# 10XGenomics/lariat

Measured on AMD Instinct MI355X. Metric: read-pairs/sec aligned to hg38 (per-barcode align loop: SMEM seeding + SW + RFA/MAPQ on device); synthetic hg38-scale reference, higher is better.
Workload: dtype u64/i32 (FM-index + integer DP), f64 (RFA scores)

## Files before the change

include/lariat_hip.h:

```cpp
#ifndef LARIAT_HIP_H
#define LARIAT_HIP_H

#include <stddef.h>
#include <stdint.h>

#ifdef __cplusplus
extern "C" {
#endif

#define LH_ABI_VERSION 6

#define LH_OK 0
#define LH_E_ARG 1
#define LH_E_IO 2
#define LH_E_HIP 3
#define LH_E_CAPACITY 4
#define LH_E_NODEVICE 5
#define LH_E_LIMIT 6

#define LH_MAX_READ_LEN 250

typedef struct lh_index lh_index;
typedef struct lh_context lh_context;

typedef struct lh_opts {
    int32_t abi_version;
    int32_t a, b, o_del, e_del, o_ins, e_ins;
    int32_t pen_unpaired, pen_clip5, pen_clip3;
    int32_t w, zdrop, T;
    int32_t min_seed_len, min_chain_weight, max_chain_extend;
    float split_factor;
    int32_t split_width, max_occ, max_chain_gap, max_ins;
    float mask_level, drop_ratio, XA_drop_ratio, mask_level_redun;
    float mapQ_coef_len;
    int32_t max_mem_intv, max_matesw;
    int32_t pes_low, pes_high;
    int32_t rescue_score_delta;
    int32_t rescue_max_hits;
    int32_t aln_score_delta;
    double improper_pair_penalty;
    double genome_length;
    int32_t run_inference;
    uint32_t flags;
} lh_opts;

#define LH_F_NO_SWEEP_FILTER 1u
#define LH_F_EXT_WAVE 16u
#define LH_F_EXT_SERIAL 32u
#define LH_F_P2_TASKS 128u
#define LH_F_RESCUE_FULL 256u
#define LH_F_CHAIN_WAVE 64u

typedef struct lh_index_opts {
    int32_t abi_version;
    int32_t sa_intv;
    int32_t sb_shift;
    int32_t no_kmer_table;
    int32_t no_unique_runs;
    int32_t no_sweep_filter;
    int32_t build_chunk_log2;
    int32_t ktree_levels;
} lh_index_opts;
void lh_index_opts_init(lh_index_opts* io);

typedef struct lh_context_opts {
    int32_t abi_version;
    int32_t smem_grid;
    int32_t aln_grid;
    int32_t rfa_grid;
    int32_t rfa_slab_kb;
    int32_t lanes;
    int32_t big_slots;
    int32_t rfa_tier_kb[2];
    int32_t rfa_tier_grid[2];
    int32_t seed_budget_kb;
} lh_context_opts;
void lh_context_opts_init(lh_context_opts* co);

typedef struct lh_batch {
    int32_t n_barcodes;
    int32_t n_pairs;
    const int32_t* bc_pair_off;
    const uint8_t* bc_do_rfa;
    const int64_t* seq_off;
    const uint8_t* seq;
    const uint64_t* name_seed;
    const int64_t* cen_start;
    const int64_t* cen_end;
} lh_batch;

typedef struct lh_result {
    int32_t abi_version;
    int32_t n_reads;
    int64_t n_cand;
    const int64_t* cand_off;
    const int32_t* rid;
    const int64_t* pos;
    const int64_t* aend;
    const int64_t* rb;
    const int64_t* re;
    const uint8_t* reversed;
    const int32_t* score;
    const int32_t* qb;
// ... 210 lines not shown
```

lariat_amd/capi.py:

```python
import ctypes as C
import os

import numpy as np

_HERE = os.path.dirname(os.path.abspath(__file__))
LIB_PATH = os.environ.get("LARIAT_HIP_LIB") or os.path.join(_HERE, "_build", "liblariat_hip.so")

LH_OK = 0
LH_ABI_VERSION = 6
LH_E_ARG, LH_E_IO, LH_E_HIP, LH_E_CAPACITY, LH_E_NODEVICE, LH_E_LIMIT = 1, 2, 3, 4, 5, 6
LH_REC_DEBUG_TAGS = 1
LH_F_NO_SWEEP_FILTER, LH_F_EXT_WAVE, LH_F_EXT_SERIAL, LH_F_CHAIN_WAVE, LH_F_P2_TASKS, LH_F_RESCUE_FULL = 1, 16, 32, 64, 128, 256
LH_MAX_READ_LEN = 250

c_i32p = C.POINTER(C.c_int32)
c_i64p = C.POINTER(C.c_int64)
c_u8p = C.POINTER(C.c_uint8)
c_u32p = C.POINTER(C.c_uint32)
c_u64p = C.POINTER(C.c_uint64)
c_f64p = C.POINTER(C.c_double)


class LhOpts(C.Structure):
    _fields_ = [
        ("abi_version", C.c_int32),
        ("a", C.c_int32), ("b", C.c_int32), ("o_del", C.c_int32), ("e_del", C.c_int32), ("o_ins", C.c_int32), ("e_ins", C.c_int32),
        ("pen_unpaired", C.c_int32), ("pen_clip5", C.c_int32), ("pen_clip3", C.c_int32),
        ("w", C.c_int32), ("zdrop", C.c_int32), ("T", C.c_int32),
        ("min_seed_len", C.c_int32), ("min_chain_weight", C.c_int32), ("max_chain_extend", C.c_int32),
        ("split_factor", C.c_float),
        ("split_width", C.c_int32), ("max_occ", C.c_int32), ("max_chain_gap", C.c_int32), ("max_ins", C.c_int32),
        ("mask_level", C.c_float), ("drop_ratio", C.c_float), ("XA_drop_ratio", C.c_float), ("mask_level_redun", C.c_float),
        ("mapQ_coef_len", C.c_float),
        ("max_mem_intv", C.c_int32), ("max_matesw", C.c_int32),
        ("pes_low", C.c_int32), ("pes_high", C.c_int32),
        ("rescue_score_delta", C.c_int32), ("rescue_max_hits", C.c_int32), ("aln_score_delta", C.c_int32),
        ("improper_pair_penalty", C.c_double), ("genome_length", C.c_double),
        ("run_inference", C.c_int32), ("flags", C.c_uint32),
    ]


class LhIndexOpts(C.Structure):
    _fields_ = [("abi_version", C.c_int32), ("sa_intv", C.c_int32), ("sb_shift", C.c_int32), ("no_kmer_table", C.c_int32), ("no_unique_runs", C.c_int32),
                ("no_sweep_filter", C.c_int32), ("build_chunk_log2", C.c_int32), ("ktree_levels", C.c_int32)]


class LhContextOpts(C.Structure):
    _fields_ = [("abi_version", C.c_int32), ("smem_grid", C.c_int32), ("aln_grid", C.c_int32), ("rfa_grid", C.c_int32), ("rfa_slab_kb", C.c_int32),
                ("lanes", C.c_int32), ("big_slots", C.c_int32), ("rfa_tier_kb", C.c_int32 * 2), ("rfa_tier_grid", C.c_int32 * 2), ("seed_budget_kb", C.c_int32)]


class LhRoundInfo(C.Structure):
    _fields_ = [("n_rounds", C.c_int32), ("max_barcode", C.c_int32), ("first_barcode", c_i32p), ("round_seeds", c_i64p), ("round_need_bytes", c_i64p),
                ("need_bytes", C.c_int64), ("budget_bytes", C.c_int64), ("max_barcode_need_bytes", C.c_int64)]


class LhBatch(C.Structure):
    _fields_ = [
        ("n_barcodes", C.c_int32), ("n_pairs", C.c_int32),
        ("bc_pair_off", c_i32p), ("bc_do_rfa", c_u8p),
        ("seq_off", c_i64p), ("seq", c_u8p), ("name_seed", c_u64p),
        ("cen_start", c_i64p), ("cen_end", c_i64p),
    ]


# ... 888 lines not shown
```

lariat_amd/csrc/k_seed.h:

```cpp
#pragma once
#include "lh_dev.h"

struct DSeed { i64 rbeg; int32_t qbeg, len; };

#define LH_SCAN_TILE 2048
__device__ __forceinline__ i64 scan_val(const int32_t* in, int i, int n, int add, int at_least) {
    if (i >= n) return 0;
    i64 v = (i64)in[i] + add;
    return v < at_least ? at_least : v;
}
__global__ void __launch_bounds__(256) k_scan_partial(int n, const int32_t* __restrict__ in, int add, int at_least, i64* __restrict__ tile_sum) {
    __shared__ i64 part[256];
    int t = threadIdx.x, base = blockIdx.x * LH_SCAN_TILE + t * 8;
    i64 s = 0;
    for (int u = 0; u < 8; ++u) s += scan_val(in, base + u, n, add, at_least);
    part[t] = s;
    __syncthreads();
    for (int d = 128; d >= 1; d >>= 1) {
        if (t < d) part[t] += part[t + d];
        __syncthreads();
    }
    if (t == 0) tile_sum[blockIdx.x] = part[0];
}
__global__ void __launch_bounds__(256) k_scan_tiles(int n_tiles, i64* __restrict__ tile_sum) {
    __shared__ i64 part[256];
    __shared__ i64 carry_s;
    int t = threadIdx.x;
    if (t == 0) carry_s = 0;
    __syncthreads();
    for (int base = 0; base < n_tiles; base += 256) {
        int i = base + t;
        i64 v = i < n_tiles ? tile_sum[i] : 0;
        part[t] = v;
        __syncthreads();
        for (int d = 1; d < 256; d <<= 1) {
            i64 o = t >= d ? part[t - d] : 0;
            __syncthreads();
            part[t] += o;
            __syncthreads();
        }
        i64 excl = part[t] - v + carry_s;
        __syncthreads();
        if (i < n_tiles) tile_sum[i] = excl;
        if (t == 255) carry_s += part[255];
        __syncthreads();
    }
    if (t == 0) tile_sum[n_tiles] = carry_s;
}
__global__ void __launch_bounds__(256) k_scan_final(int n, const int32_t* __restrict__ in, int add, int at_least, const i64* __restrict__ tile_sum, int n_tiles,
                                                    i64* __restrict__ out) {
    __shared__ i64 part[256];
    int t = threadIdx.x, base = blockIdx.x * LH_SCAN_TILE + t * 8;
    i64 loc[8], s = 0;
    for (int u = 0; u < 8; ++u) { loc[u] = s; s += scan_val(in, base + u, n, add, at_least); }
    part[t] = s;
    __syncthreads();
    for (int d = 1; d < 256; d <<= 1) {
        i64 o = t >= d ? part[t - d] : 0;
        __syncthreads();
        part[t] += o;
        __syncthreads();
    }
    i64 excl = part[t] - s + tile_sum[blockIdx.x];
    for (int u = 0; u < 8; ++u) if (base + u < n) out[base + u] = excl + loc[u];
    if (blockIdx.x == 0 && t == 0) out[n] = tile_sum[n_tiles];
}

__global__ void __launch_bounds__(256) k_seed_owner(int n_reads, const i64* __restrict__ seed_off, i64 pool_cap, int32_t* __restrict__ owner) {
    for (int r = blockIdx.x * blockDim.x + threadIdx.x; r < n_reads; r += gridDim.x * blockDim.x) {
        i64 e = seed_off[r + 1] < pool_cap ? seed_off[r + 1] : pool_cap;
        for (i64 g = seed_off[r]; g < e; ++g) owner[g] = r;
    }
}

__global__ void __launch_bounds__(256) k_seed(DIndex ix, DOpts o, int n_reads, const i64* __restrict__ seed_off, i64 pool_cap,
                                              const DIntv* __restrict__ intv, const int32_t* __restrict__ n_intv, DSeed* __restrict__ seeds,
                                              int32_t* __restrict__ s_rid, DCounters* __restrict__ ctr, const int32_t* __restrict__ owner,
                                              const int32_t* __restrict__ big_slot, const DIntv* __restrict__ big_slab) {
    i64 total = seed_off[n_reads];
    if (total > pool_cap) total = pool_cap;
    i64 stride = (i64)gridDim.x * blockDim.x;
    i64 nrounds = (total + stride - 1) / stride;
    for (i64 rd = 0; rd < nrounds; ++rd) {
        i64 g = rd * stride + (i64)blockIdx.x * blockDim.x + threadIdx.x;
        int nlf = 0, nsa = 0;
        if (g < total) {
            int r = owner[g];
            i64 u = g - seed_off[r];
            const int bs = big_slot ? big_slot[r] : -1;
            const DIntv* iv = bs < 0 ? intv + (size_t)r * LH_MAX_INTV : big_slab + ((size_t)bs * 2 + 1) * LH_BIG_INTV;
            int n = n_intv[r];
            u64 x0 = 0, step = 1, info = 0;
            for (int t = 0; t < n; ++t) {
                u64 s = iv[t].x2;
                u64 st = 1, c = s;
                if (s > (u64)o.max_occ) {
                    st = s / (u64)o.max_occ;
                    c = (s + st - 1) / st;
                    if (c > (u64)o.max_occ) c = (u64)o.max_occ;
                }
                if ((u64)u < c) { x0 = iv[t].x0; step = st; info = iv[t].info; break; }
                u -= (i64)c;
            }
            i64 rbeg;
            if (x0 >> 62 & 1) rbeg = (i64)(x0 & ~(1ull << 62));
            else rbeg = (i64)dev_sa(ix, x0 + (u64)u * step, &nlf);
            nsa = 1;
            int qbeg = (int)(info >> 32), slen = (int)(uint32_t)info - qbeg;
            DSeed sd;
            sd.rbeg = rbeg; sd.qbeg = qbeg; sd.len = slen;
            seeds[g] = sd;
            s_rid[g] = dev_intv2rid(ix, rbeg, rbeg + slen);
        }
        if (ctr) {
            int tl = wave_sum_i32(nlf), ts = wave_sum_i32(nsa);
            if (LANE() == 0 && ts) { atomicAdd(&LH_CTR(ctr)->n_lf, (u64)tl); atomicAdd(&LH_CTR(ctr)->n_sa, (u64)ts); }
        }
    }
}
```

lariat_amd/csrc/lh_dev.h:

```cpp
#pragma once
#include <stdint.h>

#ifdef LH_EMU
#include "hip_emu.h"
#define LH_LAUNCH(kernel, grid, block, stream, ...)                                          \
    do {                                                                                     \
        if (getenv("LH_EMU_TRACE")) fprintf(stderr, "emu launch %s grid=%d\n", #kernel, (int)(grid)); \
        emu::launch(dim3(grid), dim3(block), [&]() { kernel(__VA_ARGS__); });                \
    } while (0)
struct uint4 { uint32_t x, y, z, w; };
struct uint2 { uint32_t x, y; };
#else
#include <hip/hip_runtime.h>
#define LH_LAUNCH(kernel, grid, block, stream, ...) \
    hipLaunchKernelGGL(kernel, dim3(grid), dim3(block), 0, stream, __VA_ARGS__)
#endif

#define LH_WAVE 64
#define LH_MAXLEN 250
#ifndef LH_MAX_INTV
#define LH_MAX_INTV 64
#endif
#define LH_BIG_INTV 1024
#define LH_MAX_CIGAR 64
// ... 72 lines not shown
    int32_t min_seed_len, min_chain_weight, max_chain_extend, split_width, max_occ, max_chain_gap, max_ins, max_mem_intv, max_matesw;
    float split_factor, mask_level, drop_ratio, XA_drop_ratio, mask_level_redun, mapQ_coef_len;
    int32_t pes_low, pes_high, rescue_score_delta, rescue_max_hits, aln_score_delta, run_inference;
    double improper_pair_penalty, genome_length;
    int8_t mat[25];
    int32_t* wd;
};

struct DIntv { u64 x0, x1, x2, info; };

struct DReg {
    i64 rb, re;
    int32_t qb, qe, rid, score, truesc, sub, csub, w, seedcov, secondary, seedlen0, n_comp, is_alt;
    float frac_rep;
};

#define LH_CTR_SLOTS 64
struct DCounters { u64 n_ext, n_lf, n_sa, win_bases, n_chain_ext, ext_cells, glob_cells, n_rescue, rescue_cells, n_ext_exec[3], n_ktree[3], n_bt, rescue_cells_exec, n_glob_listed, n_glob_exec; };
#define LH_CTR(ctr) ((ctr) + (blockIdx.x & (LH_CTR_SLOTS - 1)))

__device__ __forceinline__ u64 shfl_u64(u64 v, int src) {
    uint32_t lo = (uint32_t)v, hi = (uint32_t)(v >> 32);
    lo = __shfl(lo, src); hi = __shfl(hi, src);
    return (u64)hi << 32 | lo;
}
__device__ __forceinline__ i64 shfl_i64(i64 v, int src) { return (i64)shfl_u64((u64)v, src); }
__device__ __forceinline__ i64 shfl_xor_i64(i64 v, int m) {
    uint32_t lo = (uint32_t)(u64)v, hi = (uint32_t)((u64)v >> 32);
    lo = __shfl_xor(lo, m); hi = __shfl_xor(hi, m);
    return (i64)((u64)hi << 32 | lo);
}
#ifdef LH_EMU
__device__ __forceinline__ int wave_max_i32(int v) {
    for (int m = 32; m >= 1; m >>= 1) { int o = __shfl_xor(v, m); v = v > o ? v : o; }
    return v;
}
__device__ __forceinline__ int wave_min_i32(int v) {
    for (int m = 32; m >= 1; m >>= 1) { int o = __shfl_xor(v, m); v = v < o ? v : o; }
    return v;
}
__device__ __forceinline__ int wave_sum_i32(int v) {
    for (int m = 32; m >= 1; m >>= 1) v += __shfl_xor(v, m);
    return v;
}
__device__ __forceinline__ int wave_scan_max_i32(int v, int lane) {
    for (int d = 1; d < 64; d <<= 1) { int o = __shfl_up(v, d); if (lane >= d) v = v > o ? v : o; }
    return v;
}
__device__ __forceinline__ int wave_scan_add_i32(int v) {
    int lane = LANE();
    for (int d = 1; d < 64; d <<= 1) { int o = __shfl_up(v, d); if (lane >= d) v += o; }
    return v;
}
__device__ __forceinline__ int wave_shr1_i32(int v, int fill) { int o = __shfl_up(v, 1); return LANE() == 0 ? fill : o; }
__device__ __forceinline__ int wave_readlane(int v, int l) { return __shfl(v, l); }
#else
#define LH_DPP(old, v, ctrl, rmask) __builtin_amdgcn_update_dpp((old), (v), (ctrl), (rmask), 0xF, false)
__device__ __forceinline__ int wave_scan_max_i32(int v, int) {
    const int ID = (int)0x80000000;
    int t;
    t = LH_DPP(ID, v, 0x111, 0xF); v = v > t ? v : t;
    t = LH_DPP(ID, v, 0x112, 0xF); v = v > t ? v : t;
    t = LH_DPP(ID, v, 0x114, 0xF); v = v > t ? v : t;
    t = LH_DPP(ID, v, 0x118, 0xF); v = v > t ? v : t;
    t = LH_DPP(ID, v, 0x142, 0xA); v = v > t ? v : t;
    t = LH_DPP(ID, v, 0x143, 0xC); v = v > t ? v : t;
    return v;
}
__device__ __forceinline__ int wave_readlane(int v, int l) { return __builtin_amdgcn_readlane(v, __builtin_amdgcn_readfirstlane(l)); }
__device__ __forceinline__ int wave_shr1_i32(int v, int fill) { return LH_DPP(fill, v, 0x138, 0xF); }
__device__ __forceinline__ int wave_max_i32(int v) { return wave_readlane(wave_scan_max_i32(v, 0), 63); }
__device__ __forceinline__ int wave_min_i32(int v) { return -wave_max_i32(-v); }
__device__ __forceinline__ int wave_scan_add_i32(int v) {
    v += LH_DPP(0, v, 0x111, 0xF);
    v += LH_DPP(0, v, 0x112, 0xF);
    v += LH_DPP(0, v, 0x114, 0xF);
    v += LH_DPP(0, v, 0x118, 0xF);
    v += LH_DPP(0, v, 0x142, 0xA);
    v += LH_DPP(0, v, 0x143, 0xC);
    return v;
}
__device__ __forceinline__ int wave_sum_i32(int v) {
    v += LH_DPP(0, v, 0x111, 0xF);
    v += LH_DPP(0, v, 0x112, 0xF);
    v += LH_DPP(0, v, 0x114, 0xF);
    v += LH_DPP(0, v, 0x118, 0xF);
    v += LH_DPP(0, v, 0x142, 0xA);
    v += LH_DPP(0, v, 0x143, 0xC);
    return wave_readlane(v, 63);
}
#endif
#ifdef LH_EMU
__device__ __forceinline__ i64 wave_max_i64(i64 v) { for (int m = 32; m >= 1; m >>= 1) { i64 o = shfl_xor_i64(v, m); v = v > o ? v : o; } return v; }
__device__ __forceinline__ i64 wave_min_i64(i64 v) { for (int m = 32; m >= 1; m >>= 1) { i64 o = shfl_xor_i64(v, m); v = v < o ? v : o; } return v; }
#else
#define LH_DPP64_STEP(ctrl, rmask, id_hi, id_lo, cmp)                                                       \
    {                                                                                                      \
        const int lo_ = LH_DPP((int)(id_lo), (int)(uint32_t)(u64)v, ctrl, rmask);                          \
        const int hi_ = LH_DPP((int)(id_hi), (int)((u64)v >> 32), ctrl, rmask);                            \
        const i64 t_ = (i64)((u64)(uint32_t)hi_ << 32 | (u64)(uint32_t)lo_);                               \
        v = v cmp t_ ? v : t_;                                                                             \
    }
__device__ __forceinline__ i64 wave_max_i64(i64 v) {
    LH_DPP64_STEP(0x111, 0xF, 0x80000000u, 0u, >) LH_DPP64_STEP(0x112, 0xF, 0x80000000u, 0u, >) LH_DPP64_STEP(0x114, 0xF, 0x80000000u, 0u, >)
    LH_DPP64_STEP(0x118, 0xF, 0x80000000u, 0u, >) LH_DPP64_STEP(0x142, 0xA, 0x80000000u, 0u, >) LH_DPP64_STEP(0x143, 0xC, 0x80000000u, 0u, >)
    return (i64)((u64)(uint32_t)wave_readlane((int)((u64)v >> 32), 63) << 32 | (u64)(uint32_t)wave_readlane((int)(uint32_t)(u64)v, 63));
}
__device__ __forceinline__ i64 wave_min_i64(i64 v) {
    LH_DPP64_STEP(0x111, 0xF, 0x7fffffffu, 0xffffffffu, <) LH_DPP64_STEP(0x112, 0xF, 0x7fffffffu, 0xffffffffu, <) LH_DPP64_STEP(0x114, 0xF, 0x7fffffffu, 0xffffffffu, <)
    LH_DPP64_STEP(0x118, 0xF, 0x7fffffffu, 0xffffffffu, <) LH_DPP64_STEP(0x142, 0xA, 0x7fffffffu, 0xffffffffu, <) LH_DPP64_STEP(0x143, 0xC, 0x7fffffffu, 0xffffffffu, <)
    return (i64)((u64)(uint32_t)wave_readlane((int)((u64)v >> 32), 63) << 32 | (u64)(uint32_t)wave_readlane((int)(uint32_t)(u64)v, 63));
}
#endif
__device__ __forceinline__ int lanes_below(u64 mask, int lane) { return __popcll(mask & ((1ull << lane) - 1)); }

#ifdef LH_EMU
__device__ __forceinline__ uint32_t dpp_xor1(uint32_t v) { return __shfl_xor(v, 1); }
__device__ __forceinline__ uint32_t dpp_xor2(uint32_t v) { return __shfl_xor(v, 2); }
__device__ __forceinline__ uint32_t dpp_half_mirror(uint32_t v) { return __shfl(v, (LANE() & ~7) | (7 - (LANE() & 7))); }
__device__ __forceinline__ uint32_t dpp_ror8(uint32_t v) { return __shfl_xor(v, 8); }
#else
__device__ __forceinline__ uint32_t dpp_xor1(uint32_t v) { return (uint32_t)__builtin_amdgcn_update_dpp(0, (int)v, 0xB1, 0xF, 0xF, true); }
__device__ __forceinline__ uint32_t dpp_xor2(uint32_t v) { return (uint32_t)__builtin_amdgcn_update_dpp(0, (int)v, 0x4E, 0xF, 0xF, true); }
__device__ __forceinline__ uint32_t dpp_half_mirror(uint32_t v) { return (uint32_t)__builtin_amdgcn_update_dpp(0, (int)v, 0x141, 0xF, 0xF, true); }
__device__ __forceinline__ uint32_t dpp_ror8(uint32_t v) { return (uint32_t)__builtin_amdgcn_update_dpp(0, (int)v, 0x128, 0xF, 0xF, true); }
#endif

#define LH_BLOOM_K 19
__device__ __forceinline__ void dev_bloom_slot(u64 key, uint32_t n_words, uint32_t* word, u64* mask) {
    u64 h = key * 0x9E3779B97F4A7C15ull;
    *word = __umulhi((uint32_t)(h >> 32), n_words);
    uint32_t g = (uint32_t)(h >> 16) * 0x85EBCA6Bu;
// ... 231 lines not shown
```

lariat_amd/csrc/lh_host.inc:

```
#include <math.h>
#include <stdlib.h>
#include <stdio.h>
#include <string.h>

#include <algorithm>
#include <array>
#include <functional>
#include <memory>
#include <mutex>
#include <string>
#include <vector>
#include <deque>
#include <map>

#include "../../include/lariat_hip.h"
#include "k_smem4.h"
#include "k_chain_lane.h"
#include "k_chain_cl.h"
#include "k_rfa.h"
#include "k_rescue3.h"
#include "k_rounds.h"
#include "lh_result_cols.h"

static void lh_print_wd(const int32_t* d_wd) {
// ... 339 lines not shown
        DALLOC(g, v.bc_pair_off, (size_t)b->n_barcodes + 1); DALLOC(g, v.bc_do_rfa, (size_t)b->n_barcodes); DALLOC(g, v.cen_start, nc); DALLOC(g, v.cen_end, nc);
        sl.cap_bases = cap_bases; sl.cap_reads = n_reads; sl.cap_bc = b->n_barcodes;
    }
    v.n_pairs = b->n_pairs; v.n_reads = n_reads; v.n_bc = b->n_barcodes; v.n_bases = nb; v.max_len = (int)lmax;
    HIPCHK(hipMemcpyAsync(v.seq, b->seq, (size_t)nb, hipMemcpyHostToDevice, us));
    HIPCHK(hipMemcpyAsync(v.seq_off, b->seq_off, (size_t)(n_reads + 1) * 8, hipMemcpyHostToDevice, us));
    std::vector<u64> seeds;
    const u64* ns = (const u64*)b->name_seed;
    if (!ns) { seeds.assign(b->n_pairs, 1); ns = seeds.data(); }
    HIPCHK(hipMemcpyAsync(v.name_seed, ns, (size_t)b->n_pairs * 8, hipMemcpyHostToDevice, us));
    HIPCHK(hipMemcpyAsync(v.bc_pair_off, b->bc_pair_off, (size_t)(b->n_barcodes + 1) * 4, hipMemcpyHostToDevice, us));
    std::vector<uint8_t> rfa;
    const uint8_t* pr = b->bc_do_rfa;
    if (!pr) { rfa.assign(b->n_barcodes, 1); pr = rfa.data(); }
    HIPCHK(hipMemcpyAsync(v.bc_do_rfa, pr, (size_t)b->n_barcodes, hipMemcpyHostToDevice, us));
    v.has_cen = b->cen_start && b->cen_end;
    std::vector<i64> neg(nc, -1);
    HIPCHK(hipMemcpyAsync(v.cen_start, v.has_cen ? b->cen_start : neg.data(), nc * 8, hipMemcpyHostToDevice, us));
    HIPCHK(hipMemcpyAsync(v.cen_end, v.has_cen ? b->cen_end : neg.data(), nc * 8, hipMemcpyHostToDevice, us));
    HIPCHK(hipStreamSynchronize(us));
    std::lock_guard<std::mutex> g(c->slot_mu);
    sl.filled = true;
    if (!staged) {
        select_slot(c, sl);
        c->sel_slot = slot;
        c->resident = true; c->ran = false;
    }
    return LH_OK;
}


static int pipe_select(lh_context* c, int32_t slot) {
    if (!c) return set_err(LH_E_ARG, "lh_batch_select: null context");
    std::lock_guard<std::mutex> g(c->slot_mu);
    if (slot < 0 || (size_t)slot >= c->slots.size() || !c->slots[(size_t)slot].filled) return set_err(LH_E_ARG, "lh_batch_select: no batch resident in that slot");
    select_slot(c, c->slots[(size_t)slot]);
    c->sel_slot = slot;
    c->resident = true; c->ran = false;
    return LH_OK;
}

#define T_BEGIN(name) do { c->tnames[t] = name; HIPCHK(hipEventRecord(c->ev[t], c->stream)); } while (0)
#define T_END()                                                                                  \
    do {                                                                                         \
        if (lh_debug_sync()) {                                                                   \
            fprintf(stderr, "[lh] launched %s ...", c->tnames[t]); fflush(stderr);               \
            hipError_t e_ = hipStreamSynchronize(c->stream);                                     \
            fprintf(stderr, " done (%s)\n", e_ == hipSuccess ? "ok" : hipGetErrorString(e_)); fflush(stderr); \
            lh_print_wd(c->d_wd);                                                                    \
        }                                                                                        \
        ++t;                                                                                     \
    } while (0)

static int run_scan(lh_context* c, int n, const int32_t* in, int add, int at_least, i64* out) {
    int nt = (n + LH_SCAN_TILE - 1) / LH_SCAN_TILE;
    LH_LAUNCH(k_scan_partial, nt, 256, c->stream, n, in, add, at_least, c->d_tile_sum);
    LH_LAUNCH(k_scan_tiles, 1, 256, c->stream, nt, c->d_tile_sum);
    LH_LAUNCH(k_scan_final, nt, 256, c->stream, n, in, add, at_least, c->d_tile_sum, nt, out);
    return LH_OK;
}

static ExtArgs ext_args(lh_context* c) {
    ExtArgs A;
    A.seq = c->b.seq; A.q4 = c->q4; A.seq_off = c->b.seq_off; A.seed_off = c->d_seed_off; A.chains = c->d_chains; A.cseeds = c->d_cseeds; A.n_chains = c->d_n_chains;
    A.sorder = c->d_srt; A.sdone = c->d_ord; A.chain_rmax = c->d_chain_rmax; A.reg_off = c->d_reg_off; A.regs = c->d_regs; A.n_regs = c->d_n_regs; A.est = c->d_ext_st;
    const ExtUnits U(c->d_ext_u, (size_t)c->pool_cap);
    A.nreg_u = U.nreg_u; A.u_read = U.u_read; A.est_u = U.est_u; A.rflag = ExtLongLists(c->d_ext_long, (size_t)c->cap_reads).rflag;
    return A;
}

#include "lh_host_trace.inc"

template <int PASS, bool BIG, int QW = 32> static void smem_pass(lh_context* c, const DIndex& ix4, const DOpts& o, int N, int grid, const K1Big& big) {
    int32_t* const next = BIG ? &c->d_next_read->big_pass[PASS - 1] : &c->d_next_read->pass[PASS - 1];
    LH_LAUNCH((k_smem_pass<PASS, BIG, QW>), grid, 64, c->stream, ix4, o, N, c->b.seq, c->b.seq_off, c->d_intv, c->d_n_intv, c->d_status, c->d_slab4, next, c->d_ctr, big);
}

static int k1_big_round(lh_context* c, const DOpts& o, const DIndex& ix4, int N, int base) {
    const int g4 = (N + 63) / 64 < c->grid_smem4 ? (N + 63) / 64 : c->grid_smem4;
    const int gb = g4 < 64 ? g4 : 64;
    HIPCHK(hipMemsetAsync(c->d_big_count, 0, sizeof(K1BigCounts), c->stream));
    HIPCHK(hipMemsetAsync(c->d_next_read->big_pass, 0, sizeof c->d_next_read->big_pass, c->stream));
    K1Big big; big.list = c->d_big_list; big.count = &c->d_big_count->listed; big.slot = c->d_big_slot; big.slab = c->d_big_slab; big.resume = nullptr;
    LH_LAUNCH(k_big_collect, (N + 255) / 256, 256, c->stream, N, c->d_status, c->d_n_intv, c->d_big_slot, c->d_big_list, &c->d_big_count->listed, base, c->big_cap - base);
    smem_pass<1, true>(c, ix4, o, N, gb, big);
    smem_pass<2, true>(c, ix4, o, N, gb, big);
    if (o.max_mem_intv > 0) smem_pass<3, true>(c, ix4, o, N, gb, big);
    LH_LAUNCH(k_smem_fin_big, gb, 64, c->stream, o, big, (const int32_t*)c->d_n_intv, c->d_seed_cnt, c->d_l_rep);
    return LH_OK;
}

static int peek_seed_total(lh_context* c, int N) {
    LH_LAUNCH(k_peek_i64_i32, 1, 1, c->stream, (const i64*)(c->d_seed_off + N), (const int32_t*)&c->d_big_count->asked, &c->h_peek->k1.seeds);
    HIPCHK(hipStreamSynchronize(c->stream));
    return LH_OK;
}

static inline int ext_long_min(int N);
static int run_front(lh_context* c, const DOpts& o, int& t) {
    int N = c->b.n_reads;
    const DIndex& ix = c->idx->d;
    HIPCHK(hipMemsetAsync(c->d_ctr, 0, sizeof(DCounters) * LH_CTR_SLOTS, c->stream));
    const uint32_t* q4 = nullptr;
    if (ix.tn) {
        LH_LAUNCH(k_pack_reads, 4096, 256, c->stream, (const uint8_t*)c->b.seq, c->b.n_bases, c->d_seq4 + 2);
        q4 = c->d_seq4 + 2;
    }
    c->q4 = q4;
    DIndex ix4 = ix;
    if (c->flags & LH_F_NO_SWEEP_FILTER) ix4.bloom1 = ix4.bloom2 = nullptr;
    {
        const int g4 = (N + 63) / 64 < c->grid_smem4 ? (N + 63) / 64 : c->grid_smem4;
        HIPCHK(hipMemsetAsync(c->d_next_read, 0, sizeof(K1Counters), c->stream));
        K1Big nobig; nobig.list = nullptr; nobig.count = nullptr; nobig.slot = nullptr; nobig.slab = nullptr; nobig.resume = nullptr;
        K1Big first = nobig; first.list = c->d_k1_todo; first.count = &c->d_next_read->n_todo; first.resume = c->d_k1_resume;
        const int g3 = (N + 63) / 64 < 2 * c->grid_smem4 ? (N + 63) / 64 : 2 * c->grid_smem4;
        T_BEGIN("k_smem4");
        LH_LAUNCH(k_smem_first, (N + 255) / 256, 256, c->stream, ix4, o, N, q4, (const i64*)c->b.seq_off, c->d_intv, c->d_n_intv, c->d_status, c->d_k1_resume, c->d_k1_todo, &c->d_next_read->n_todo, c->d_ctr);
#ifdef LH_K1_TRACE
        K1Trace trace;
        { int rc = k1_trace_begin(c, trace, g4); if (rc) return rc; }
#endif
        const bool qw_small = c->b.max_len <= 8 * LH_K1_QW_SMALL;
        if (qw_small) smem_pass<1, false, LH_K1_QW_SMALL>(c, ix4, o, N, g4, first);
        else smem_pass<1, false>(c, ix4, o, N, g4, first);
        T_END();
#ifdef LH_K1_TRACE
        { int rc = k1_trace_replay(c, trace, N, g4); if (rc) return rc; }
#endif
        T_BEGIN("k_smem4_p2");
        const bool p2_tasks = ((c->flags & LH_F_P2_TASKS) || (c->ext_hint_valid && c->h_peek->prev_wave_reads >= ext_long_min(N))) && N < (1 << 27);
        K1Big p2 = nobig;
        if (p2_tasks) {
            p2.list = c->d_p2_tasks; p2.count = &c->d_next_read->n_p2_tasks; p2.slot = c->d_k1_todo;
            LH_LAUNCH(k_p2_tasks, (N + 255) / 256, 256, c->stream, o, N, (const DIntv*)c->d_intv, (const int32_t*)c->d_n_intv, c->d_p2_tasks, &c->d_next_read->n_p2_tasks, c->d_k1_todo);
        }
        if (qw_small) smem_pass<2, false, LH_K1_QW_SMALL>(c, ix4, o, N, g4, p2);
        else smem_pass<2, false>(c, ix4, o, N, g4, p2);
        if (p2_tasks) LH_LAUNCH(k_p2_clamp, (N + 255) / 256, 256, c->stream, N, c->d_n_intv);
        T_END();
#ifdef LH_K1_TRACE
        { int rc = k1_trace_lens(c, trace); if (rc) return rc; }
#endif
        T_BEGIN("k_smem4_p3");
        if (o.max_mem_intv > 0 && q4)
            LH_LAUNCH(k_smem_p3_lock, (N + 255) / 256, 256, c->stream, ix4, o, N, q4, (const i64*)c->b.seq_off, c->d_intv, c->d_n_intv, c->d_status, c->d_ctr);
        else if (o.max_mem_intv > 0)
            smem_pass<3, false>(c, ix4, o, N, g3, nobig);
        T_END();
        T_BEGIN("k_smem_fin");
        { int rc = k1_big_round(c, o, ix4, N, 0); if (rc) return rc; }
        LH_LAUNCH(k_smem_fin, (N * 16 + 255) / 256, 256, c->stream, o, N, c->d_intv, c->d_n_intv, c->d_seed_cnt, c->d_l_rep, (const int32_t*)c->d_big_slot);
        T_END();
    }
    T_BEGIN("k_scan_seeds");
    { int rc = run_scan(c, N, c->d_seed_cnt, 0, 0, c->d_seed_off); if (rc) return rc; }
    T_END();
    {
        { int rc = peek_seed_total(c, N); if (rc) return rc; }
        while (c->h_peek->k1.big_asked > (i64)(c->big_cap - c->big_base)) {
            const i64 asked = c->h_peek->k1.big_asked, old_cap = c->big_cap, new_cap = old_cap + asked + asked / 8 + 16;
            if (new_cap > (1 << 30)) return set_err(LH_E_CAPACITY, "too many reads with more than LH_MAX_INTV SMEM intervals for one batch: split the batch");
            DIntv* slab = nullptr; int32_t* list = nullptr;
            DevGroup grown;
            DALLOC(grown, slab, (size_t)new_cap * 2 * LH_BIG_INTV); DALLOC(grown, list, (size_t)new_cap);
            HIPCHK(hipMemcpyAsync(slab, c->d_big_slab, (size_t)old_cap * 2 * LH_BIG_INTV * sizeof(DIntv), hipMemcpyDeviceToDevice, c->stream));
            HIPCHK(hipStreamSynchronize(c->stream));
            std::swap(c->d_big_slab, slab); std::swap(c->d_big_list, list);
            grown.release();
            c->big_base = (int)old_cap; c->big_cap = (int)new_cap;
            { int rc = k1_big_round(c, o, ix4, N, c->big_base); if (rc) return rc; }
            { int rc = run_scan(c, N, c->d_seed_cnt, 0, 0, c->d_seed_off); if (rc) return rc; }
            { int rc = peek_seed_total(c, N); if (rc) return rc; }
        }
        c->big_base = 0;
        const i64 total = c->h_peek->k1.seeds;
        if (!c->in_round) c->rounds.total_seeds = total;
        if (total > c->pool_cap || c->co.seed_budget_kb > 0) {
            const i64 need = seed_need(c, total);
            i64 budget = 0;
            { int rc = seed_budget(c, &budget); if (rc) return rc; }
            if (!c->in_round) c->rounds.budget = budget;
            if (need > budget) {
                if (!c->dump_stop_after_dedup && !c->in_round) return LH_NEED_ROUNDS;
                return set_err(LH_E_CAPACITY, "the batch has " + std::to_string(total) + " seeds: their workspace (" + std::to_string((long long)(need / 1000000000)) + " GB) does not fit the " +
                                                  std::to_string((long long)(budget / 1000000000)) + " GB of its budget (seed_budget_kb, or the HBM that is free): split the batch");
            }
            if (total > c->pool_cap) {
                int rc = alloc_seed_pools(c, total + total / 4);
                if (rc) return rc;
            }
        }
    }
    T_BEGIN("k_seed");
    int g2 = (int)((i64)N * 8 / 256 + 1); if (g2 > 2048) g2 = 2048;
    LH_LAUNCH(k_seed_owner, (N + 255) / 256 < 8192 ? (N + 255) / 256 : 8192, 256, c->stream, N, (const i64*)c->d_seed_off, c->pool_cap, c->d_s_next);
    LH_LAUNCH(k_seed, g2, 256, c->stream, ix, o, N, c->d_seed_off, c->pool_cap, c->d_intv, c->d_n_intv, c->d_seeds, c->d_s_rid, c->d_ctr, (const int32_t*)c->d_s_next, (const int32_t*)c->d_big_slot, (const DIntv*)c->d_big_slab);
    T_END();
    T_BEGIN("k_scan_regs");
    { int rc = run_scan(c, N, c->d_seed_cnt, LH_RESCUE_SLOTS, 0, c->d_reg_off); if (rc) return rc; }
    T_END();
    T_BEGIN("k_chain");
    HIPCHK(hipMemsetAsync(c->d_ext_jobs, 0, sizeof(DExtJobs), c->stream));
    {
        ExtArgs A = ext_args(c);
        const int fuse = (c->flags & LH_F_EXT_WAVE) ? 0 : 1;
        LH_LAUNCH(k_chain_lane, (N + 63) / 64, 64, c->stream, ix, o, N, c->pool_cap, c->d_seeds, c->d_s_rid, c->d_l_rep, c->d_chains, c->d_cseeds, c->d_n_chains, c->d_status,
                  c->d_aln_r, c->d_ext_jobs->wave_range + 1, c->d_srt, c->d_chain_rmax, c->d_ctr, A, fuse, c->d_ext_jobs->count + 1, c->d_ext_jlist, c->d_ext_jkey,
                  c->d_ext_jobs->heavy_range + 1, c->d_ext_heavy);
        const int32_t* wlist = c->d_aln_r;
        const int32_t* wcount = c->d_ext_jobs->wave_range + 1;
        if (!(c->flags & LH_F_CHAIN_WAVE)) {
            int32_t* const fb_count = &c->d_aln_count->full;
            HIPCHK(hipMemsetAsync(fb_count, 0, sizeof(int32_t), c->stream));
#define LH_K3_CL(CAP_, GRID_, LO_, LAST_, ST_)                                                                                                                         \
            LH_LAUNCH((k_chain_cl<CAP_>), N < (GRID_) ? N : (GRID_), 64, ST_, ix, o, (const i64*)c->b.seq_off, (const i64*)c->d_seed_off, c->pool_cap, (const DSeed*)c->d_seeds, \
                      (const int32_t*)c->d_s_rid, (const int32_t*)c->d_l_rep, c->d_chains, c->d_cseeds, c->d_n_chains, c->d_status, wlist, wcount, LO_, LAST_, c->d_aln_ci, fb_count)
            HIPCHK(hipEventRecord(c->ev_fork, c->stream));
            HIPCHK(hipStreamWaitEvent(c->aux[1], c->ev_fork, 0)); HIPCHK(hipStreamWaitEvent(c->aux[2], c->ev_fork, 0));
            LH_K3_CL(LH_CHAIN_CL_CAP_C, 2048, LH_CHAIN_CL_CAP_B, 1, c->aux[2]);
            LH_K3_CL(LH_CHAIN_CL_CAP_B, 8192, LH_CHAIN_CL_CAP_A, 0, c->aux[1]);
            LH_K3_CL(LH_CHAIN_CL_CAP_A, 16384, 0, 0, c->stream);
            HIPCHK(hipEventRecord(c->ev_join[1], c->aux[1])); HIPCHK(hipEventRecord(c->ev_join[2], c->aux[2]));
            HIPCHK(hipStreamWaitEvent(c->stream, c->ev_join[1], 0)); HIPCHK(hipStreamWaitEvent(c->stream, c->ev_join[2], 0));
#undef LH_K3_CL
            wlist = c->d_aln_ci; wcount = fb_count;
#ifdef LH_RFA_PROF
            { int rc = prof_chain_cl(c); if (rc) return rc; }
#endif
            if (lh_debug_sync()) {
                int32_t nl = 0, nf = 0;
                if (hipStreamSynchronize(c->stream) == hipSuccess && hipMemcpy(&nl, c->d_ext_jobs->wave_range + 1, 4, hipMemcpyDeviceToHost) == hipSuccess &&
                    hipMemcpy(&nf, fb_count, 4, hipMemcpyDeviceToHost) == hipSuccess)
                    fprintf(stderr, "[lh] K3: %d reads listed for the wave kernels, %d of them left to k_chain by k_chain_cl\n", nl, nf);
            }
        }
        LH_LAUNCH(k_chain, N < 16384 ? N : 16384, 64, c->stream, ix, o, N, c->b.seq_off, c->d_seed_off, c->pool_cap, c->d_seeds, c->d_s_rid, c->d_l_rep, c->d_s_next, c->d_ct,
                  c->d_ord, c->d_srt, c->d_chains, c->d_cseeds, c->d_n_chains, c->d_status, wlist, wcount);
    }
    T_END();
    return LH_OK;
}

static int round_mem_for(lh_context* c, int n_bc, bool view, i64 n_reads, i64 n_bases) {
    RoundBufs& rb = c->rb;
    if (n_bc > rb.cap_bc || (view && (n_reads > rb.cap_reads || n_bases > rb.cap_bases))) {
        HIPCHK(hipStreamSynchronize(c->stream));
        c->round_mem.release();
        const bool v = view || rb.cap_reads > 0;
        const i64 cb = n_bc > rb.cap_bc ? n_bc : rb.cap_bc, cr = !v ? 0 : n_reads > rb.cap_reads ? n_reads : rb.cap_reads, cs = !v ? 0 : n_bases > rb.cap_bases ? n_bases : rb.cap_bases;
        rb = RoundBufs();
        DevGroup& g = c->round_mem;
        DALLOC(g, rb.prefix, cb + 1);
// ... 91 lines not shown
            if (pending) { c->dl_pending = true; c->dl_finish = std::move(finish); }
        }
    } restore{c, whole, host_pending, host_finish};
    c->in_round = true;
    lh_result* acc = nullptr;
    for (i64 r = 0; r < n_rounds; ++r) {
        const int b0 = (int)P.cut_bc()[r], p0 = (int)P.cut_pair()[r];
        const i64 s0 = P.cut_base()[r];
        const BatchView part = part_view(whole, c->rb, P, r);
        int rt = 0;
        HIPCHK(hipEventRecord(c->ev[LH_NSTAGE - 1], c->stream));
        {
            const i64 work = part.n_bases / 8 > part.n_reads ? part.n_bases / 8 : part.n_reads;
            LH_LAUNCH(k_batch_view, (int)(work / 256 + 1 < 4096 ? work / 256 + 1 : 4096), 256, c->stream, part.n_bc, part.n_reads, part.n_bases, b0, p0, s0, (const int32_t*)whole.bc_pair_off,
                      (const i64*)whole.seq_off, (const uint8_t*)whole.seq, c->rb.v_bc_pair_off, c->rb.v_seq_off, c->rb.v_seq);
        }
        HIPCHK(hipEventRecord(c->ev[LH_NSTAGE], c->stream));
        c->b = part;
        int rc = run_front(c, o, rt);
        if (!rc) rc = stage2_run(c, o, rt);
        lh_result* res = nullptr;
        if (!rc) {
            hipError_t e = hipEventRecord(c->ev[rt], c->stream);
            if (e == hipSuccess) e = hipStreamSynchronize(c->stream);
            if (e != hipSuccess) rc = set_err(LH_E_HIP, std::string("round ") + std::to_string(r) + ": " + hipGetErrorString(e));
        }
        if (!rc) rc = add_times(c, rt, sums, nullptr);
        if (!rc) { float v = 0; hipEventElapsedTime(&v, c->ev[LH_NSTAGE - 1], c->ev[LH_NSTAGE]); sums.add("k_batch_view", v); }
        if (!rc) {
            c->ran = true;
            rc = pipe_download(c, &res);
            c->ran = false;
            if (rc) rc = set_err(rc, "round " + std::to_string(r) + " of " + std::to_string(n_rounds) + " (its reads start at read " + std::to_string(2 * (i64)p0) + " of the batch): " + g_err);
        }
        if (!rc) rc = merge_into(acc, res);
        if (rc) {
            const std::string why = g_err;
            quiesce(c);
            if (acc) lh_result_free(acc);
            return set_err(rc, why);
        }
    }
    c->round_result = acc;
    R.n_rounds = (int)n_rounds;
    c->n_t = sums.n;
    for (int i = 0; i < sums.n; ++i) { c->tnames[i] = sums.names[i]; c->tms[i] = sums.ms[i]; }
    return LH_OK;
}

static int pipe_align(lh_context* c, const lh_opts* opts) {
    if (!c || !opts) return set_err(LH_E_ARG, "lh_align_resident: null argument");
    if (!c->resident) return set_err(LH_E_ARG, "no batch resident: call lh_batch_upload first");
    if (opts->abi_version != LH_ABI_VERSION) return set_err(LH_E_ARG, "lh_opts.abi_version does not match LH_ABI_VERSION (use lh_opts_init)");
    if (opts->flags & ~(LH_F_NO_SWEEP_FILTER | LH_F_EXT_WAVE | LH_F_EXT_SERIAL | LH_F_CHAIN_WAVE | LH_F_P2_TASKS | LH_F_RESCUE_FULL)) return set_err(LH_E_ARG, "lh_opts.flags: unknown bit set");
    HIPCHK(hipSetDevice(c->idx->device));
    {
        std::vector<void*> fl;
        { std::lock_guard<std::mutex> g(c->slot_mu); fl.swap(c->free_later); }
        for (void* q : fl) hipFree(q);
    }
    if (c->round_result) { lh_result_free(c->round_result); c->round_result = nullptr; }
    c->rounds.clear();
    c->ran = false;
    if (!c->pool_cap) { int rc = alloc_seed_pools(c, first_pool_cap(c)); if (rc) return rc; }
    if (!c->cand_cap) { int rc = alloc_cand_pools(c, first_cand_cap(c)); if (rc) return rc; }
    DOpts o = to_dopts(opts);
    o.wd = c->d_wd;
    c->flags = opts->flags;
    int t = 0;
    int rc = run_front(c, o, t);
    const bool in_rounds = rc == LH_NEED_ROUNDS;
    if (in_rounds) rc = align_rounds(c, o, t);
    else if (!rc) rc = stage2_run(c, o, t);
    if (rc) { quiesce(c); return rc; }
    if (!in_rounds) {
        HIPCHK(hipEventRecord(c->ev[t], c->stream));
        HIPCHK(hipStreamSynchronize(c->stream));
        HIPCHK(hipGetLastError());
        c->n_t = t;
        for (int i = 0; i < t; ++i) HIPCHK(hipEventElapsedTime(&c->tms[i], c->ev[i], c->ev[i + 1]));
        c->rounds.n_rounds = 1;
    }
    c->ran = true;
    return LH_OK;
}

int lh_last_timings(lh_context* c, int32_t* n, const char* const** names, const float** ms) {
    if (!c) return set_err(LH_E_ARG, "null context");
    if (n) *n = c->n_t;
    if (names) *names = c->tnames;
    if (ms) *ms = c->tms;
    return LH_OK;
}

struct DumpArenaH {
    lh_stage_dump d;
    std::vector<i64> intv_off, seed_off, seed_rbeg, chain_off, chain_pos, reg_off, reg_rb, reg_re;
    std::vector<u64> intv;
    std::vector<int32_t> seed_qbeg, seed_len, seed_rid, chain_nseeds, chain_rid, chain_w, chain_kept, reg_qb, reg_qe, reg_rid, reg_score, reg_truesc,
        reg_w, reg_seedcov, reg_seedlen0, reg_csub, reg_secondary;
};

template <class T> static int d2h(std::vector<T>& v, const T* d, size_t n) {
    v.resize(n);
    if (n && hipMemcpy(v.data(), d, n * sizeof(T), hipMemcpyDeviceToHost) != hipSuccess) return set_err(LH_E_HIP, "hipMemcpy D2H failed");
    return LH_OK;
}
// ... 76 lines not shown
```

Before: 49.68 million.

## Expand seeds per read group with row-scan and fuse region-offset scan

Replaces the per-seed owner-map plus flat seed kernel with a wave-per-4-reads kernel. Each 16-lane row scans a read's interval counts with DPP row prefix sums and expands the seeds cooperatively. It also fuses the region-offset scan into the seed-offset scan by emitting a second output with a per-index constant added. This drops the k_seed_owner pass and a separate three-kernel scan, in exchange for more shared-memory traffic and possible imbalance when reads have very different seed counts. The old path stays available behind a new flag.

```diff
diff --git a/include/lariat_hip.h b/include/lariat_hip.h
--- a/include/lariat_hip.h
+++ b/include/lariat_hip.h
@@ -8,7 +8,7 @@
 extern "C" {
 #endif
 
-#define LH_ABI_VERSION 6
+#define LH_ABI_VERSION 7
 
 #define LH_OK 0
 #define LH_E_ARG 1
@@ -49,6 +49,7 @@
 #define LH_F_EXT_SERIAL 32u
 #define LH_F_P2_TASKS 128u
 #define LH_F_RESCUE_FULL 256u
+#define LH_F_SEED_LANE 512u
 #define LH_F_CHAIN_WAVE 64u
 
 typedef struct lh_index_opts {
diff --git a/lariat_amd/capi.py b/lariat_amd/capi.py
--- a/lariat_amd/capi.py
+++ b/lariat_amd/capi.py
@@ -7,10 +7,10 @@
 LIB_PATH = os.environ.get("LARIAT_HIP_LIB") or os.path.join(_HERE, "_build", "liblariat_hip.so")
 
 LH_OK = 0
-LH_ABI_VERSION = 6
+LH_ABI_VERSION = 7
 LH_E_ARG, LH_E_IO, LH_E_HIP, LH_E_CAPACITY, LH_E_NODEVICE, LH_E_LIMIT = 1, 2, 3, 4, 5, 6
 LH_REC_DEBUG_TAGS = 1
-LH_F_NO_SWEEP_FILTER, LH_F_EXT_WAVE, LH_F_EXT_SERIAL, LH_F_CHAIN_WAVE, LH_F_P2_TASKS, LH_F_RESCUE_FULL = 1, 16, 32, 64, 128, 256
+LH_F_NO_SWEEP_FILTER, LH_F_EXT_WAVE, LH_F_EXT_SERIAL, LH_F_CHAIN_WAVE, LH_F_P2_TASKS, LH_F_RESCUE_FULL, LH_F_SEED_LANE = 1, 16, 32, 64, 128, 256, 512
 LH_MAX_READ_LEN = 250
 
 c_i32p = C.POINTER(C.c_int32)
diff --git a/lariat_amd/csrc/k_seed.h b/lariat_amd/csrc/k_seed.h
--- a/lariat_amd/csrc/k_seed.h
+++ b/lariat_amd/csrc/k_seed.h
@@ -48,7 +48,7 @@
     if (t == 0) tile_sum[n_tiles] = carry_s;
 }
 __global__ void __launch_bounds__(256) k_scan_final(int n, const int32_t* __restrict__ in, int add, int at_least, const i64* __restrict__ tile_sum, int n_tiles,
-                                                    i64* __restrict__ out) {
+                                                    i64* __restrict__ out, i64* __restrict__ out2, int add2) {
     __shared__ i64 part[256];
     int t = threadIdx.x, base = blockIdx.x * LH_SCAN_TILE + t * 8;
     i64 loc[8], s = 0;
@@ -64,6 +64,10 @@
     i64 excl = part[t] - s + tile_sum[blockIdx.x];
     for (int u = 0; u < 8; ++u) if (base + u < n) out[base + u] = excl + loc[u];
     if (blockIdx.x == 0 && t == 0) out[n] = tile_sum[n_tiles];
+    if (out2) {
+        for (int u = 0; u < 8; ++u) if (base + u < n) out2[base + u] = excl + loc[u] + (i64)(base + u) * add2;
+        if (blockIdx.x == 0 && t == 0) out2[n] = tile_sum[n_tiles] + (i64)n * add2;
+    }
 }
 
 __global__ void __launch_bounds__(256) k_seed_owner(int n_reads, const i64* __restrict__ seed_off, i64 pool_cap, int32_t* __restrict__ owner) {
@@ -118,3 +122,83 @@
         }
     }
 }
+
+__device__ __forceinline__ u64 dev_seed_step(const DOpts& o, u64 s, u64* step) {
+    *step = 1;
+    if (s <= (u64)o.max_occ) return s;
+    const u64 st = s / (u64)o.max_occ, c = (s + st - 1) / st;
+    *step = st;
+    return c < (u64)o.max_occ ? c : (u64)o.max_occ;
+}
+
+struct K2Intv { u64 x0, x2, info; };
+__device__ __forceinline__ K2Intv k2_load(const DIntv* __restrict__ iv, int e, int n) {
+    K2Intv m;
+    m.x0 = m.x2 = m.info = 0;
+    if (e < n) { m.x0 = iv[e].x0; m.x2 = iv[e].x2; m.info = iv[e].info; }
+    return m;
+}
+#define LH_K2_GRID 16384
+__global__ void __launch_bounds__(64) k_seed_grp(DIndex ix, DOpts o, int n_reads, const i64* __restrict__ seed_off, i64 pool_cap, const DIntv* __restrict__ intv,
+                                                 const int32_t* __restrict__ n_intv, DSeed* __restrict__ seeds, int32_t* __restrict__ s_rid, DCounters* __restrict__ ctr,
+                                                 const int32_t* __restrict__ big_slot, const DIntv* __restrict__ big_slab) {
+    __shared__ u64 sh_x0[64], sh_info[64], sh_step[64];
+    __shared__ int sh_incl[64];
+    const int lane = LANE(), sub = lane & 15, row = lane & ~15;
+    const int n_items = (n_reads + 3) >> 2;
+    int nlf = 0, nsa = 0;
+    for (int item = blockIdx.x; item < n_items; item += gridDim.x) {
+        const int r = item * 4 + (lane >> 4);
+        const bool live = r < n_reads;
+        int n = 0, S = 0;
+        i64 base = 0;
+        const DIntv* iv = intv;
+        if (live) {
+            n = n_intv[r];
+            base = seed_off[r];
+            const i64 end = seed_off[r + 1] < pool_cap ? seed_off[r + 1] : pool_cap;
+            S = end > base ? (int)(end - base) : 0;
+            const int bs = big_slot ? big_slot[r] : -1;
+            iv = bs < 0 ? intv + (size_t)r * LH_MAX_INTV : big_slab + ((size_t)bs * 2 + 1) * LH_BIG_INTV;
+        }
+        const int n_chunks = wave_max_i32((n + 15) >> 4);
+        int run = 0;
+        for (int ch = 0; ch < n_chunks; ++ch) {
+            const bool have = ch * 16 + sub < n;
+            const K2Intv m = k2_load(iv, ch * 16 + sub, n);
+            u64 m_step = 1;
+            const int cnt = have ? (int)dev_seed_step(o, m.x2, &m_step) : 0;
+            EMU_SYNC();
+            sh_x0[lane] = m.x0; sh_info[lane] = m.info; sh_step[lane] = m_step; sh_incl[lane] = row_scan_add_i32(cnt);
+            EMU_SYNC();
+            const int tot = sh_incl[row | 15];
+            const int n_iter = wave_max_i32((tot + 15) >> 4);
+            for (int it = 0; it < n_iter; ++it) {
+                const int k = it * 16 + sub;
+                int j = 0;
+#pragma unroll
+                for (int w = 8; w >= 1; w >>= 1) j += sh_incl[row | (j + w - 1)] <= k ? w : 0;
+                const int src = row | j;
+                if (k < tot && run + k < S) {
+                    const int u = k - (j ? sh_incl[src - 1] : 0);
+                    const u64 x0 = sh_x0[src], st = sh_step[src], info = sh_info[src];
+                    i64 rbeg;
+                    if (x0 >> 62 & 1) rbeg = (i64)(x0 & ~(1ull << 62));
+                    else { int lf = 0; rbeg = (i64)dev_sa(ix, x0 + (u64)u * st, &lf); nlf += lf; }
+                    ++nsa;
+                    const int qbeg = (int)(info >> 32), slen = (int)(uint32_t)info - qbeg;
+                    DSeed sd;
+                    sd.rbeg = rbeg; sd.qbeg = qbeg; sd.len = slen;
+                    const i64 g = base + run + k;
+                    seeds[g] = sd;
+                    s_rid[g] = dev_intv2rid(ix, rbeg, rbeg + slen);
+                }
+            }
+            run += tot;
+        }
+    }
+    if (ctr) {
+        const int tl = wave_sum_i32(nlf), ts = wave_sum_i32(nsa);
+        if (lane == 0 && ts) { atomicAdd(&LH_CTR(ctr)->n_lf, (u64)tl); atomicAdd(&LH_CTR(ctr)->n_sa, (u64)ts); }
+    }
+}
diff --git a/lariat_amd/csrc/lh_dev.h b/lariat_amd/csrc/lh_dev.h
--- a/lariat_amd/csrc/lh_dev.h
+++ b/lariat_amd/csrc/lh_dev.h
@@ -148,6 +148,11 @@
     for (int d = 1; d < 64; d <<= 1) { int o = __shfl_up(v, d); if (lane >= d) v += o; }
     return v;
 }
+__device__ __forceinline__ int row_scan_add_i32(int v) {
+    int sub = LANE() & 15;
+    for (int d = 1; d < 16; d <<= 1) { int o = __shfl_up(v, d); if (sub >= d) v += o; }
+    return v;
+}
 __device__ __forceinline__ int wave_shr1_i32(int v, int fill) { int o = __shfl_up(v, 1); return LANE() == 0 ? fill : o; }
 __device__ __forceinline__ int wave_readlane(int v, int l) { return __shfl(v, l); }
 #else
@@ -174,6 +179,13 @@
     v += LH_DPP(0, v, 0x118, 0xF);
     v += LH_DPP(0, v, 0x142, 0xA);
     v += LH_DPP(0, v, 0x143, 0xC);
+    return v;
+}
+__device__ __forceinline__ int row_scan_add_i32(int v) {
+    v += LH_DPP(0, v, 0x111, 0xF);
+    v += LH_DPP(0, v, 0x112, 0xF);
+    v += LH_DPP(0, v, 0x114, 0xF);
+    v += LH_DPP(0, v, 0x118, 0xF);
     return v;
 }
 __device__ __forceinline__ int wave_sum_i32(int v) {
diff --git a/lariat_amd/csrc/lh_host.inc b/lariat_amd/csrc/lh_host.inc
--- a/lariat_amd/csrc/lh_host.inc
+++ b/lariat_amd/csrc/lh_host.inc
@@ -415,11 +415,11 @@
         ++t;                                                                                     \
     } while (0)
 
-static int run_scan(lh_context* c, int n, const int32_t* in, int add, int at_least, i64* out) {
+static int run_scan(lh_context* c, int n, const int32_t* in, int add, int at_least, i64* out, i64* out2 = nullptr, int add2 = 0) {
     int nt = (n + LH_SCAN_TILE - 1) / LH_SCAN_TILE;
     LH_LAUNCH(k_scan_partial, nt, 256, c->stream, n, in, add, at_least, c->d_tile_sum);
     LH_LAUNCH(k_scan_tiles, 1, 256, c->stream, nt, c->d_tile_sum);
-    LH_LAUNCH(k_scan_final, nt, 256, c->stream, n, in, add, at_least, c->d_tile_sum, nt, out);
+    LH_LAUNCH(k_scan_final, nt, 256, c->stream, n, in, add, at_least, c->d_tile_sum, nt, out, out2, add2);
     return LH_OK;
 }
 
@@ -517,7 +517,7 @@
         T_END();
     }
     T_BEGIN("k_scan_seeds");
-    { int rc = run_scan(c, N, c->d_seed_cnt, 0, 0, c->d_seed_off); if (rc) return rc; }
+    { int rc = run_scan(c, N, c->d_seed_cnt, 0, 0, c->d_seed_off, c->d_reg_off, LH_RESCUE_SLOTS); if (rc) return rc; }
     T_END();
     {
         { int rc = peek_seed_total(c, N); if (rc) return rc; }
@@ -533,7 +533,7 @@
             grown.release();
             c->big_base = (int)old_cap; c->big_cap = (int)new_cap;
             { int rc = k1_big_round(c, o, ix4, N, c->big_base); if (rc) return rc; }
-            { int rc = run_scan(c, N, c->d_seed_cnt, 0, 0, c->d_seed_off); if (rc) return rc; }
+            { int rc = run_scan(c, N, c->d_seed_cnt, 0, 0, c->d_seed_off, c->d_reg_off, LH_RESCUE_SLOTS); if (rc) return rc; }
             { int rc = peek_seed_total(c, N); if (rc) return rc; }
         }
         c->big_base = 0;
@@ -556,12 +556,15 @@
         }
     }
     T_BEGIN("k_seed");
-    int g2 = (int)((i64)N * 8 / 256 + 1); if (g2 > 2048) g2 = 2048;
-    LH_LAUNCH(k_seed_owner, (N + 255) / 256 < 8192 ? (N + 255) / 256 : 8192, 256, c->stream, N, (const i64*)c->d_seed_off, c->pool_cap, c->d_s_next);
-    LH_LAUNCH(k_seed, g2, 256, c->stream, ix, o, N, c->d_seed_off, c->pool_cap, c->d_intv, c->d_n_intv, c->d_seeds, c->d_s_rid, c->d_ctr, (const int32_t*)c->d_s_next, (const int32_t*)c->d_big_slot, (const DIntv*)c->d_big_slab);
-    T_END();
-    T_BEGIN("k_scan_regs");
-    { int rc = run_scan(c, N, c->d_seed_cnt, LH_RESCUE_SLOTS, 0, c->d_reg_off); if (rc) return rc; }
+    if (c->flags & LH_F_SEED_LANE) {
+        int g2 = (int)((i64)N * 8 / 256 + 1); if (g2 > 2048) g2 = 2048;
+        LH_LAUNCH(k_seed_owner, (N + 255) / 256 < 8192 ? (N + 255) / 256 : 8192, 256, c->stream, N, (const i64*)c->d_seed_off, c->pool_cap, c->d_s_next);
+        LH_LAUNCH(k_seed, g2, 256, c->stream, ix, o, N, c->d_seed_off, c->pool_cap, c->d_intv, c->d_n_intv, c->d_seeds, c->d_s_rid, c->d_ctr, (const int32_t*)c->d_s_next, (const int32_t*)c->d_big_slot, (const DIntv*)c->d_big_slab);
+    } else {
+        const int items = (N + 3) / 4;
+        LH_LAUNCH(k_seed_grp, items < LH_K2_GRID ? items : LH_K2_GRID, 64, c->stream, ix, o, N, (const i64*)c->d_seed_off, c->pool_cap, (const DIntv*)c->d_intv, (const int32_t*)c->d_n_intv, c->d_seeds, c->d_s_rid, c->d_ctr,
+                  (const int32_t*)c->d_big_slot, (const DIntv*)c->d_big_slab);
+    }
     T_END();
     T_BEGIN("k_chain");
     HIPCHK(hipMemsetAsync(c->d_ext_jobs, 0, sizeof(DExtJobs), c->stream));
@@ -759,7 +762,7 @@
     if (!c || !opts) return set_err(LH_E_ARG, "lh_align_resident: null argument");
     if (!c->resident) return set_err(LH_E_ARG, "no batch resident: call lh_batch_upload first");
     if (opts->abi_version != LH_ABI_VERSION) return set_err(LH_E_ARG, "lh_opts.abi_version does not match LH_ABI_VERSION (use lh_opts_init)");
-    if (opts->flags & ~(LH_F_NO_SWEEP_FILTER | LH_F_EXT_WAVE | LH_F_EXT_SERIAL | LH_F_CHAIN_WAVE | LH_F_P2_TASKS | LH_F_RESCUE_FULL)) return set_err(LH_E_ARG, "lh_opts.flags: unknown bit set");
+    if (opts->flags & ~(LH_F_NO_SWEEP_FILTER | LH_F_EXT_WAVE | LH_F_EXT_SERIAL | LH_F_CHAIN_WAVE | LH_F_P2_TASKS | LH_F_RESCUE_FULL | LH_F_SEED_LANE)) return set_err(LH_E_ARG, "lh_opts.flags: unknown bit set");
     HIPCHK(hipSetDevice(c->idx->device));
     {
         std::vector<void*> fl;
```

Result: faster. 50.95 million, median of 6 (+2.5%).
